# SahakyanLab/GenomeAssembler_dev

Measured on AMD Instinct MI355X. Metric: k-mers built+scored/sec, higher is better.
Workload: dtype u64 keys / u32 counts / f64 scores; 1 GPU; cfg2 (configs[2]): 100 x 50000 bp segments per GPU, 150 bp reads at 50x, k=31, build + breakage scoring of all contigs; mode=segments, segments_total=100, distinct_kmers_rank0=3843627, parallelism=segments sharded over 1 GPU(s), no collective

## Files before the change

genomeassembler_dev_amd/csrc/kernels.h:

```cpp
#pragma once
#include <hip/hip_runtime.h>
#include <stdint.h>

#include "device_utils.h"
#include "keyops.h"

struct ReadSet {
    const u64* words;
    const u64* read_off;
    const u64* seg_read_off;
    const u32* seg_tile_start;
    const uint4* tile_info;
    u32 fixed_len;
    u32 n_segments;
};

__device__ __forceinline__ void read_span(const ReadSet& rs, u64 r, u64* p0, u32* len) {
    if (rs.fixed_len) { *p0 = rs.read_off ? rs.read_off[r] : r * rs.fixed_len; *len = rs.fixed_len; }
    else { const u64 a = rs.read_off[r]; *p0 = a; *len = (u32)(rs.read_off[r + 1] - a); }
}

struct GraphView {
    const void* dk_key;
    const u32* dstart;
// ... 7 lines not shown
__device__ __forceinline__ u32 graph_lower_bound(const GraphView& gv, u32 seg, const K& t, u32* bucket_hi) {
    const K* dk = reinterpret_cast<const K*>(gv.dk_key);
    const u32 nb = 1u << gv.bbits;
    const int low = 2 * gv.k - gv.bbits;
    const u32 gb = seg * nb + (gv.bbits ? kfield(t, low) : 0u);
    uint2 dd;
    __builtin_memcpy(&dd, gv.dstart + gb, 8);
    const u32 base = dd.x;
    *bucket_hi = dd.y;
    const int bshift = low > gv.fbits ? low - gv.fbits : 0;
    const u32 nbin = 1u << gv.fbits;
    const u16* f = gv.fdir + (u64)gb * (nbin + 1) + (kfield(t, bshift) & (nbin - 1));
    u32 ff;
    __builtin_memcpy(&ff, f, 4);
    u32 lo = base + (ff & 0xFFFFu);
    u32 hi = base + (ff >> 16);
    if (hi > *bucket_hi) hi = *bucket_hi;
    if (lo > hi) lo = hi;
    while (hi - lo > 4) {
        const u32 m = (lo + hi) >> 1;
        if (kless(dk[m], t)) lo = m + 1;
        else hi = m;
    }
    while (lo < hi && kless(dk[lo], t)) ++lo;
    return lo;
}

struct PathSet {
    const u64* words;
    const u64* p_off;
    const u32* seg_path_off;
    u32 n_segments;
};

#define GASM_KT 16
#define GASM_SCORE_PATH_CAP 6144
#define GASM_TBL 4096
#define GASM_TBL_LIMIT 2816

__global__ void k_pack_ascii(const u8* ascii, u64 nbases_host, const u64* nbases_dev, u64* words, u32* err);
#define GASM_TILE_WG 512
template <class K> __global__ void k_tile_hist(ReadSet rs, const uint4* tinfo, int k, int bbits, u32 g, u32 n_tiles, ushort4* tcnt);
__global__ void k_tile_scan(ReadSet rs, int bbits, u32 padm, const ushort4* tcnt, u32* toff, u32* hist, u32* flags);
template <class TO> __global__ void k_scan_excl(const u32* in, TO* out, u32 n);
__global__ void k_copy_u64(const u64* a, u64* b, u32 n);
template <class K>
__global__ void k_bucket_scatter(ReadSet rs, const uint4* tinfo, int k, int bbits, u32 g, u32 padm, u32 n_tiles, const u64* bstart, const u32* toff,
                                 const ushort4* tcnt, K* keys, u64 scratch);
#define GASM_RT_MAX 16
template <class K>
__global__ void k_bucket_partition(ReadSet rs, const uint4* tinfo, int k, int bbits, u32 g, u32 padm, u32 n_tiles, const u64* bstart, u32* cursor,
                                   K* keys, u64 scratch, u32* flags);
template <class K, int TBL>
__global__ void k_bucket_dedup(K* keys, u32* mult, const u64* bstart, const u32* blen, u32* bucket_d, u32* overflow, u16* fdir, int low_bits, int dbg,
                               unsigned long long* stamps, u32* dstart);
#define GASM_BUCKET_MAX 65535
template <class K>
__global__ void k_bucket_dedup_multi(const K* keys, K* keys_out, u32* mult, const u64* bstart, u32* bucket_d, u32* overflow, u16* fdir, int low_bits);
template <class K>
__global__ void k_bucket_gather(const K* keys, const u32* mult, const u64* bstart, const u32* dstart, K* dk_key, u32* dk_cnt, u32* claim, u8* eflag,
                                u32* flags);
template <class K> __global__ void k_edge_target(GraphView gv, u32 n_segments, u32 chunks, u32* tgt, u32* claim);
__global__ void k_edge_multi(GraphView gv, u32 n_segments, u32 chunks, const u32* tgt, const u32* claim, u8* eflag);
template <class K>
__global__ void k_node_flags(GraphView gv, u32 n_segments, u32 chunks, const u32* claim, u8* eflag, u64* link, u32* clen);
__global__ void k_edge_next(GraphView gv, u32 n_segments, u32 chunks, const u32* tgt, const u8* eflag, u32* nxt, u64* link);
__global__ void k_link_jump(GraphView gv, u32 n_segments, u32 chunks, u64* link, const u32* prev_active, u32* active, int jumps, const u32* nxt,
                            u32* clen);
__global__ void k_rank_rulers(GraphView gv, u32 n_segments, u32 chunks, u64* link, u32* rtab, u32 rshift, u32* flags);
__global__ void k_rank_lds(GraphView gv, const u32* rtab, u64* link, int max_rounds, u32 rshift, u32 lds_entries, u32* flags);
__global__ void k_chain_len(const u32* nxt, const u64* link, u32* clen, const u32* n_edges_p);
__global__ void k_contig_scan(GraphView gv, const u8* eflag, const u32* clen, u32* e_cid, u64* e_coff, u32* seg_ncontig,
                              u64* seg_cbases, u32* done, u32* seg_cstart, u64* seg_bstart, const u32* flags, u32* report, u32 ticket);
__global__ void k_contig_place(GraphView gv, const u8* eflag, const u32* seg_cstart, const u64* seg_bstart, u32* e_cid, u64* e_coff,
                               u64* c_off, u32 n_segments, u32 chunks);
template <class K>
__global__ void k_contig_emit(GraphView gv, const u64* link, const u32* nxt, const u64* e_coff, u8* out, u32 n_segments, u32 chunks);

template <class K>
__global__ void k_pack_runs(const K* keys, const u32* mult, const u64* bstart, const u32* bucket_d, const u32* gb_list, const u64* dst_off, K* out_keys,
                            u32* out_cnt);
template <class K, int TBL>
__global__ void k_bucket_merge(const K* in_keys, const u32* in_cnt, const u64* run_off, const u32* run_len, u32 n_src, K* out_keys, u32* out_cnt,
                               const u64* bstart, u32* bucket_d, u32* overflow, u16* fdir, int low_bits, const u64* src_base);
__global__ void k_repack_reads(const u64* src, const u64* dir, u64* words_out);
__global__ void k_piece_positions(const u64* piece_first, const u64* piece_word_off, u32 n_pieces, u64 n_reads, u32 fixed_len, u64* pos);
__global__ void k_slice_last(const u32* a, const u64* off, u32 n, u32* out);

__global__ void k_chain_expand(const u64* cwords, const u64* c_off, const u64* sig_off, const u32* elem_contig, const u32* elem_skip, const u64* elem_pos,
                               const u64* out_off, u32 n_scaffolds, u64* out, u64 n_words);
struct ChainSigs {
    const u64* sig_off;
    const u32* elem_contig;
    const u32* elem_skip;
    const u64* elem_pos;
};
__global__ void k_str_bitonic(const u64* words, const u64* off, u32* idx, u32 n_pow2, u32 kk, u32 j, ChainSigs cs);
__global__ void k_str_bitonic_block(const u64* words, const u64* off, u32* idx, u32 n_pow2, u32 kk, u32 j0, ChainSigs cs);
__global__ void k_str_adjacent_eq(const u64* words, const u64* off, const u32* idx, u32 n, u8* same_as_prev, ChainSigs cs);
__global__ void k_unpack_ascii(const u64* words, u64 nbases, u8* out);
__global__ void k_guided_chain(PathSet ps, const unsigned long long* fx, int k, u32* g_next, u32* g_prev, u32* dbg_order);
__global__ void k_asm_match(const u64* cwords, const u64* c_off, u32 n, int k, u8* match, u8* row_any, u8* level_any);
__global__ void k_asm_merge(const u32* perm, u32 rows, u32 n, int k, const u32* clen, const u8* match, const u8* row_any, const u8* level_any,
                            const u64* cwords, const u64* c_off, u32* out_next, u8* out_ov, u32* out_heads, u32* out_nchains, u8* need_host);

__global__ void k_sim_weights(const u64* gwords, const u64* gbase, const u64* woff, u32 n_segments, int kmer, const long long* fixw, u64* w);
template <class T> __global__ void k_seg_scan_incl(T* a, const u64* off);
__global__ void k_sim_draw(const u64* cum, const u64* woff, const u64* doff, const u64* glen, u64 seed, u32 read_len, u32* start, u32* keep);
// ... 47 lines not shown
```

genomeassembler_dev_amd/csrc/kernels_build.hip:

```cpp
#include "device_utils.h"
#include "keyops.h"
#include "kernels.h"
#include "dedup_order.h"

typedef unsigned long long u64x2 __attribute__((ext_vector_type(2)));

typedef unsigned int u32x4nt __attribute__((ext_vector_type(4)));
#ifndef GASM_NO_NT
__device__ __forceinline__ uint4 stream_load16(const uint4* p) {
    const u32x4nt v = __builtin_nontemporal_load(reinterpret_cast<const u32x4nt*>(p));
    return make_uint4(v.x, v.y, v.z, v.w);
}
#define GASM_STREAM_LOAD(p) stream_load16(p)
#define GASM_STREAM_STORE(v, p) __builtin_nontemporal_store((v), (p))
#else
#define GASM_STREAM_LOAD(p) (*(p))
#define GASM_STREAM_STORE(v, p) (*(p) = (v))
#endif

__global__ void __launch_bounds__(GASM_WG) k_pack_ascii(const u8* __restrict__ ascii, u64 nbases_host, const u64* __restrict__ nbases_dev,
                                                        u64* __restrict__ words, u32* __restrict__ err) {
    const u64 nbases = nbases_dev ? *nbases_dev : nbases_host;
    const u64 nwords = (nbases + 31) / 32 + 4;
    bool ok = true;
// ... 437 lines not shown

#define GASM_SLOT_LOCKED 0xFFFFFFFFu

__device__ __forceinline__ u64x2 lds_load128(const void* p) {
    __asm__ volatile("" ::: "memory");
    return *reinterpret_cast<const u64x2*>(p);
}
__device__ __forceinline__ uint4 lds_load128u(const void* p) {
    __asm__ volatile("" ::: "memory");
    return *reinterpret_cast<const uint4*>(p);
}

template <int TBL>
__device__ __forceinline__ bool dedup_step(u64* t_key, u32* t_cnt, u32* n_distinct, u64 key, u32& set) {
    constexpr u32 NSETS = TBL / 2;
    const u64x2 c = lds_load128(&t_key[2 * set]);
    int slot = c.x == key ? 0 : c.y == key ? 1 : -1;
    if (slot < 0) {
        const int emp = c.x == GASM_EMPTY64 ? 0 : c.y == GASM_EMPTY64 ? 1 : -1;
        if (emp < 0) { set = (set + 1) & (NSETS - 1); return false; }
        const u64 old = atomicCAS(reinterpret_cast<unsigned long long*>(&t_key[2 * set + emp]), (unsigned long long)GASM_EMPTY64,
                                  (unsigned long long)key);
        if (old == GASM_EMPTY64) atomicAdd(n_distinct, 1u);
        else if (old != key) return false;
        slot = emp;
    }
    atomicAdd(&t_cnt[2 * set + slot], 1u);
    return true;
}
template <int TBL>
__device__ __forceinline__ bool dedup_step(K128* t_key, u32* t_cnt, u32* n_distinct, const K128& key, u32& set) {
    constexpr u32 NSETS = TBL / 2;
    __asm__ volatile("" ::: "memory");
    const uint2 c = *reinterpret_cast<const uint2*>(&t_cnt[2 * set]);
    const u32 cc[2] = {c.x, c.y};
#pragma unroll
    for (int q = 0; q < 2; ++q) {
        if (cc[q] == GASM_SLOT_LOCKED) return false;
        if (cc[q] == 0) {
            if (atomicCAS(&t_cnt[2 * set + q], 0u, GASM_SLOT_LOCKED) != 0u) return false;
            t_key[2 * set + q] = key;
            __builtin_amdgcn_fence(__ATOMIC_RELEASE, "workgroup");
            __hip_atomic_store(&t_cnt[2 * set + q], 1u, __ATOMIC_RELAXED, __HIP_MEMORY_SCOPE_WORKGROUP);
            atomicAdd(n_distinct, 1u);
            return true;
        }
        const u64x2 kq = lds_load128(&t_key[2 * set + q]);
        if (kq.x == key.hi && kq.y == key.lo) { atomicAdd(&t_cnt[2 * set + q], 1u); return true; }
    }
    set = set + 1 >= NSETS - 1 ? 0u : set + 1;
    return false;
}

#ifndef GASM_DEDUP_NLD
#define GASM_DEDUP_NLD 3
#endif
#ifndef GASM_DEDUP_NLDW
#define GASM_DEDUP_NLDW 6
#endif
#ifndef GASM_DEDUP_WGS
#define GASM_DEDUP_WGS 6
#endif
__device__ __forceinline__ void publish_u32(u32* p, u32 v) { __hip_atomic_store(p, v, __ATOMIC_RELAXED, __HIP_MEMORY_SCOPE_AGENT); }
__device__ __forceinline__ void publish_u64(u64* p, u64 v) { __hip_atomic_store(p, v, __ATOMIC_RELAXED, __HIP_MEMORY_SCOPE_AGENT); }
__device__ __forceinline__ bool count_in_last(u32* done) {
    __asm__ volatile("s_waitcnt vmcnt(0)" ::: "memory");
    return __hip_atomic_fetch_add(done, 1u, __ATOMIC_RELAXED, __HIP_MEMORY_SCOPE_AGENT) == gridDim.x - 1;
}

__device__ __forceinline__ void dedup_last_scan(const u32* __restrict__ bucket_d, u32* __restrict__ dstart, u32 n, u32* __restrict__ done, u32* s_word,
                                                u32* s_waves ) {
    if (!dstart) return;
    __syncthreads();
    if (threadIdx.x == 0) *s_word = count_in_last(done) ? 1u : 0u;
    __syncthreads();
    if (!*s_word) return;
    const u32 per = (n + GASM_WG - 1) / GASM_WG, a = min(n, threadIdx.x * per), b = min(n, a + per);
    u32 sum = 0;
    for (u32 i = a; i < b; ++i) sum += __hip_atomic_load(&bucket_d[i], __ATOMIC_RELAXED, __HIP_MEMORY_SCOPE_AGENT);
    const u32 inc = wave_incl_scan(sum);
    __syncthreads();
    if ((threadIdx.x & 63) == 63) s_waves[threadIdx.x >> 6] = inc;
    __syncthreads();
    u32 ex = inc - sum, tot = 0;
    for (u32 w = 0; w < GASM_WG / 64; ++w) { const u32 t = s_waves[w]; if (w < (threadIdx.x >> 6)) ex += t; tot += t; }
    for (u32 i = a; i < b; ++i) { dstart[i] = ex; ex += __hip_atomic_load(&bucket_d[i], __ATOMIC_RELAXED, __HIP_MEMORY_SCOPE_AGENT); }
    if (threadIdx.x == 0) dstart[n] = tot;
}

template <class K, int TBL>
__global__ void __launch_bounds__(GASM_WG, TBL == 4096 ? 3 : sizeof(K) == 8 ? GASM_DEDUP_WGS : 4)
k_bucket_dedup(K* __restrict__ keys, u32* __restrict__ mult, const u64* __restrict__ bstart, const u32* __restrict__ blen, u32* __restrict__ bucket_d,
               u32* __restrict__ overflow, u16* __restrict__ fdir, int low_bits, int dbg, unsigned long long* __restrict__ stamps,
               u32* __restrict__ dstart) {
    constexpr int LIMIT = TBL / 16 * 11;
    constexpr int BINS = TBL / 4;
    constexpr int LOG_TBL = TBL == 4096 ? 12 : 11;
    constexpr bool WIDE = sizeof(K) == 16;
    constexpr int LOG_SETS = LOG_TBL - 1;
    constexpr u32 NSETS = 1u << LOG_SETS;
    static_assert(TBL == 4096 || TBL == 2048, "table size");
    __shared__ __align__(32) K t_key[TBL];
    __shared__ __align__(16) u32 t_cnt[TBL];
    u32 *s_tmp, *w_distinct, *w_overflow;
    if constexpr (WIDE) {
        s_tmp = reinterpret_cast<u32*>(&t_key[TBL - 2]);
        w_distinct = &t_cnt[TBL - 2];
        w_overflow = &t_cnt[TBL - 1];
    } else {
        __shared__ u32 s_tmp_narrow[8];
        s_tmp = s_tmp_narrow;
        w_distinct = &s_tmp_narrow[4];
        w_overflow = &s_tmp_narrow[5];
    }
    static_assert((TBL - LIMIT) * sizeof(K) >= 2 * BINS * sizeof(u32), "the bins must fit behind the sorted entries");
    u32* const s_start = reinterpret_cast<u32*>(t_key + LIMIT);
    u32* const s_cur = s_start + BINS;
    unsigned long long tph = stamps ? wall_clock64() : 0ull;
    auto phase = [&](int i) {
        if (stamps && threadIdx.x == 0) { const unsigned long long t = wall_clock64(); atomicAdd(&stamps[i], t - tph); tph = t; }
    };
    const u32 bucket = blockIdx.x;
    const u64 beg = bstart[bucket], end = bstart[bucket + 1];
    u64 n = end - beg;
    if (blen) {
        const u64 len = blen[bucket];
        if (len > n) {
            for (u32 i = threadIdx.x; i <= (u32)BINS; i += GASM_WG) fdir[(u64)bucket * (BINS + 1) + i] = 0;
            if (threadIdx.x == 0) publish_u32(&bucket_d[bucket], 0u);
            dedup_last_scan(bucket_d, dstart, gridDim.x, overflow + 8, s_tmp + 7, s_tmp);
            return;
        }
        n = len;
    }
    const u32 warm = (u32)(dbg >> 2) & 3u;
    for (u32 i = threadIdx.x; i < TBL; i += GASM_WG) { t_key[i] = key_empty<K>(); t_cnt[i] = 0; }
    if (!WIDE && threadIdx.x == 0) { *w_distinct = 0; *w_overflow = 0; s_tmp[6] = 0; }
    __syncthreads();
    phase(0);
    constexpr int NLD = WIDE ? GASM_DEDUP_NLDW : TBL == 2048 ? GASM_DEDUP_NLD : 4;
    constexpr int KPL = NLD * 16 / sizeof(K);
    const u64 nch = n * sizeof(K) / 16;
    const uint4* src = reinterpret_cast<const uint4*>(keys + beg);
    if (dbg & 16) src = reinterpret_cast<const uint4*>(keys + bstart[bucket & 7u]);
    uint4 v[NLD];
    auto fetch = [&](u64 c) {
#pragma unroll
        for (int q = 0; q < NLD; ++q) v[q] = c + (u64)q * GASM_WG < nch ? GASM_STREAM_LOAD(&src[c + (u64)q * GASM_WG]) : make_uint4(~0u, ~0u, ~0u, ~0u);
    };
    if (threadIdx.x < nch) fetch(threadIdx.x);
    for (u64 c = threadIdx.x; c < nch; c += NLD * GASM_WG) {
        if (c == (u64)threadIdx.x + NLD * GASM_WG) phase(1);
        K kx[KPL];
        if constexpr (WIDE) {
#pragma unroll
            for (int q = 0; q < NLD; ++q) { kx[q].hi = (u64)v[q].x | ((u64)v[q].y << 32); kx[q].lo = (u64)v[q].z | ((u64)v[q].w << 32); }
        } else {
#pragma unroll
            for (int q = 0; q < NLD; ++q) { kx[2 * q] = (u64)v[q].x | ((u64)v[q].y << 32); kx[2 * q + 1] = (u64)v[q].z | ((u64)v[q].w << 32); }
        }
        if (c + NLD * GASM_WG < nch) fetch(c + NLD * GASM_WG);
        if ((dbg & 3) == 1) { u64 x = 0; for (int q = 0; q < KPL; ++q) x ^= khash(kx[q]); if (x == 0x1234567) *w_overflow = 1; continue; }
        if (__hip_atomic_load(w_distinct, __ATOMIC_RELAXED, __HIP_MEMORY_SCOPE_WORKGROUP) > (u32)LIMIT) { *w_overflow = 1; break; }
        if constexpr (!WIDE) {
            if (c < (u64)warm * NLD * GASM_WG) {
#pragma unroll
                for (int q = 0; q < KPL; ++q) {
                    const u64 key = kx[q];
                    if (kis_filler(key)) continue;
                    u32 st = khash(key) >> (32 - LOG_SETS);
                    bool ok = false;
                    for (u32 probe = 0; probe < 8 * NSETS && !ok; ++probe) ok = dedup_step<TBL>(t_key, t_cnt, w_distinct, key, st);
                    if (!ok) *w_overflow = 1;
                }
                continue;
            }
            u32 missed = 0;
            {
                u32 set[KPL];
                u64x2 c[KPL];
#pragma unroll
                for (int q = 0; q < KPL; ++q) {
                    set[q] = khash(kx[q]) >> (32 - LOG_SETS);
                    c[q] = lds_load128(&t_key[2 * set[q]]);
                }
#pragma unroll
                for (int q = 0; q < KPL; ++q) {
                    const u64 key = kx[q];
                    if (kis_filler(key)) continue;
                    const int slot = c[q].x == key ? 0 : c[q].y == key ? 1 : -1;
                    if (slot >= 0) atomicAdd(&t_cnt[2 * set[q] + slot], 1u);
                    else missed |= 1u << q;
                }
            }
            while (missed) {
                const u32 q = (u32)__builtin_ctz(missed);
                missed &= missed - 1;
                u64 key = kx[0];
#pragma unroll
                for (u32 e = 1; e < (u32)KPL; ++e) if (e == q) key = kx[e];
                u32 st = khash(key) >> (32 - LOG_SETS);
                bool ok = false;
                for (u32 probe = 0; probe < 8 * NSETS && !ok; ++probe) ok = dedup_step<TBL>(t_key, t_cnt, w_distinct, key, st);
                if (!ok) *w_overflow = 1;
            }
        } else {
            u32 set[KPL];
            uint2 cn[KPL];
            u64x2 k0[KPL], k1[KPL];
#pragma unroll
            for (int q = 0; q < KPL; ++q) {
                set[q] = min(khash(kx[q]) >> (32 - LOG_SETS), NSETS - 2);
                __asm__ volatile("" ::: "memory");
                cn[q] = *reinterpret_cast<const uint2*>(&t_cnt[2 * set[q]]);
                k0[q] = lds_load128(&t_key[2 * set[q]]);
                k1[q] = lds_load128(&t_key[2 * set[q] + 1]);
            }
            u32 missed = 0;
#pragma unroll
            for (int q = 0; q < KPL; ++q) {
                const K128 key = kx[q];
                if (kis_filler(key)) continue;
                const bool r0 = cn[q].x != 0 && cn[q].x != GASM_SLOT_LOCKED, r1 = cn[q].y != 0 && cn[q].y != GASM_SLOT_LOCKED;
                if (r0 && k0[q].x == key.hi && k0[q].y == key.lo) atomicAdd(&t_cnt[2 * set[q]], 1u);
                else if (r0 && r1 && k1[q].x == key.hi && k1[q].y == key.lo) atomicAdd(&t_cnt[2 * set[q] + 1], 1u);
                else missed |= 1u << q;
            }
            while (missed) {
                const u32 q = (u32)__builtin_ctz(missed);
                missed &= missed - 1;
                K128 key = kx[0];
#pragma unroll
                for (u32 e = 1; e < (u32)KPL; ++e) if (e == q) key = kx[e];
                u32 st = min(khash(key) >> (32 - LOG_SETS), NSETS - 2);
                bool ok = false;
                for (u32 probe = 0; probe < 8 * NSETS && !ok; ++probe) ok = dedup_step<TBL>(t_key, t_cnt, w_distinct, key, st);
                if (!ok) *w_overflow = 1;
            }
        }
    }
    phase(2);
    __syncthreads();
    phase(3);
    if (*w_overflow || *w_distinct > (u32)LIMIT) {
        for (u32 i = threadIdx.x; i <= (u32)BINS; i += GASM_WG) fdir[(u64)bucket * (BINS + 1) + i] = 0;
        if (threadIdx.x == 0) { atomicOr(overflow, 1u); publish_u32(&bucket_d[bucket], 0u); }
        dedup_last_scan(bucket_d, dstart, gridDim.x, overflow + 8, s_tmp + 7, s_tmp);
        return;
    }
    const u32 d = *w_distinct;
    if ((dbg & 3) == 1 || (dbg & 3) == 2) { if (threadIdx.x == 0) publish_u32(&bucket_d[bucket], d); dedup_last_scan(bucket_d, dstart, gridDim.x, overflow + 8, s_tmp + 7, s_tmp); return; }
    dedup_order<K, TBL, true>(t_key, t_cnt, s_start, s_cur, s_tmp, fdir, bucket, low_bits, d);
    phase(4);
    for (u32 i = threadIdx.x; i < d; i += GASM_WG) { keys[beg + i] = t_key[i]; mult[beg + i] = t_cnt[i]; }
    if (threadIdx.x == 0) publish_u32(&bucket_d[bucket], d);
    phase(5);
    if (stamps && threadIdx.x == 0) stamps[8 + 3 * (u64)blockIdx.x + 1] = wall_clock64();
    dedup_last_scan(bucket_d, dstart, gridDim.x, overflow + 8, s_tmp + 7, s_tmp);
}
template __global__ void k_bucket_dedup<u64, 4096>(u64*, u32*, const u64*, const u32*, u32*, u32*, u16*, int, int, unsigned long long*, u32*);
template __global__ void k_bucket_dedup<u64, 2048>(u64*, u32*, const u64*, const u32*, u32*, u32*, u16*, int, int, unsigned long long*, u32*);
template __global__ void k_bucket_dedup<K128, 2048>(K128*, u32*, const u64*, const u32*, u32*, u32*, u16*, int, int, unsigned long long*, u32*);

template <class K>
__global__ void __launch_bounds__(GASM_WG) k_bucket_dedup_multi(const K* __restrict__ keys, K* __restrict__ keys_out, u32* __restrict__ mult,
                                                                const u64* __restrict__ bstart, u32* __restrict__ bucket_d,
                                                                u32* __restrict__ overflow, u16* __restrict__ fdir, int low_bits) {
    constexpr int TBL = 4096, LIMIT = TBL / 16 * 11, BINS = TBL / 4, LOG_SETS = 11, LOG_BINS = 10;
    constexpr u32 NSETS = 1u << LOG_SETS;
    __shared__ __align__(32) K t_key[TBL];
    __shared__ __align__(16) u32 t_cnt[TBL];
    __shared__ u32 s_start[BINS];
    __shared__ u32 s_cur[BINS];
    __shared__ u32 s_tmp[8];
    const u32 bucket = blockIdx.x;
    const u64 beg = bstart[bucket], n = bstart[bucket + 1] - beg;
    const int bin_bits = low_bits < LOG_BINS ? low_bits : LOG_BINS;
    const int r_max = low_bits < 16 ? low_bits : 16;
    u16* const fd = fdir + (u64)bucket * (BINS + 1);
    auto give_up = [&]() {
        for (u32 i = threadIdx.x; i <= (u32)BINS; i += GASM_WG) fd[i] = 0;
        if (threadIdx.x == 0) { atomicOr(overflow, 1u); bucket_d[bucket] = 0; }
    };
    for (int r = 0;; ++r) {
        if (r > r_max) { give_up(); return; }
        const u32 npass = 1u << r;
        u32 total = 0;
        bool fits = true;
        for (u32 p = 0; p < npass; ++p) {
            for (u32 i = threadIdx.x; i < TBL; i += GASM_WG) { t_key[i] = key_empty<K>(); t_cnt[i] = 0; }
            for (u32 i = threadIdx.x; i < BINS; i += GASM_WG) s_start[i] = 0;
            if (threadIdx.x == 0) { s_tmp[4] = 0; s_tmp[5] = 0; s_tmp[6] = 0; }
            __syncthreads();
            for (u64 i = threadIdx.x; i < n; i += GASM_WG) {
                const K key = keys[beg + i];
                if (kis_filler(key)) continue;
                if (r && (kfield(key, low_bits - r) & (npass - 1)) != p) continue;
                if (__hip_atomic_load(&s_tmp[4], __ATOMIC_RELAXED, __HIP_MEMORY_SCOPE_WORKGROUP) > (u32)LIMIT) break;
                u32 st = khash(key) >> (32 - LOG_SETS);
                bool ok = false;
                for (u32 probe = 0; probe < 8 * NSETS && !ok; ++probe) ok = dedup_step<TBL>(t_key, t_cnt, &s_tmp[4], key, st);
                if (!ok) s_tmp[5] = 1;
            }
            __syncthreads();
            const u32 d = s_tmp[4];
            if (s_tmp[5] || d > (u32)LIMIT) { fits = false; break; }
            if (total + d > GASM_BUCKET_MAX) { give_up(); return; }
            u32 lo, hi;
            if (r <= bin_bits) { lo = p << (bin_bits - r); hi = (p + 1) << (bin_bits - r); }
            else { lo = p >> (r - bin_bits); hi = (p & ((1u << (r - bin_bits)) - 1u)) ? lo : lo + 1; }
            dedup_order<K, TBL, false, true>(t_key, t_cnt, s_start, s_cur, s_tmp, fdir, bucket, low_bits, d, total, lo, hi);
            for (u32 i = threadIdx.x; i < d; i += GASM_WG) { keys_out[beg + total + i] = t_key[i]; mult[beg + total + i] = t_cnt[i]; }
            total += d;
            __syncthreads();
        }
// ... 413 lines not shown
```

genomeassembler_dev_amd/csrc/keyops.h:

```cpp
#pragma once
#include "device_utils.h"

struct __attribute__((aligned(16))) K128 {
    u64 hi, lo;
};

template <class K> __device__ __forceinline__ K key_empty();
template <> __device__ __forceinline__ u64 key_empty<u64>() { return GASM_EMPTY64; }
template <> __device__ __forceinline__ K128 key_empty<K128>() { return K128{GASM_EMPTY64, GASM_EMPTY64}; }
template <class K> __device__ __forceinline__ K key_from_u64(u64 v);
template <> __device__ __forceinline__ u64 key_from_u64<u64>(u64 v) { return v; }
template <> __device__ __forceinline__ K128 key_from_u64<K128>(u64 v) { return K128{0, v}; }

template <class K> __device__ __forceinline__ K key_filler(u32 bkt, int bshift);
__device__ __forceinline__ bool kis_filler(u64 a) { return (a >> 63) != 0; }

__device__ __forceinline__ bool keq(u64 a, u64 b) { return a == b; }
__device__ __forceinline__ bool keq(const K128& a, const K128& b) { return a.hi == b.hi && a.lo == b.lo; }
__device__ __forceinline__ bool kless(u64 a, u64 b) { return a < b; }
__device__ __forceinline__ bool kless(const K128& a, const K128& b) { return a.hi < b.hi || (a.hi == b.hi && a.lo < b.lo); }
__device__ __forceinline__ bool kis_empty(u64 a) { return a == GASM_EMPTY64; }
__device__ __forceinline__ bool kis_empty(const K128& a) { return (a.hi & a.lo) == GASM_EMPTY64; }

__device__ __forceinline__ bool kis_filler(const K128& a) { return (a.hi >> 63) != 0; }

__device__ __forceinline__ u64 kshr(u64 a, int s) { return a >> s; }
__device__ __forceinline__ K128 kshr(const K128& a, int s) {
    if (s == 0) return a;
    if (s >= 64) return K128{0, a.hi >> (s - 64)};
    return K128{a.hi >> s, (a.lo >> s) | (a.hi << (64 - s))};
}
__device__ __forceinline__ u64 kshl(u64 a, int s) { return a << s; }
__device__ __forceinline__ K128 kshl(const K128& a, int s) {
    if (s == 0) return a;
    if (s >= 64) return K128{a.lo << (s - 64), 0};
    return K128{(a.hi << s) | (a.lo >> (64 - s)), a.lo << s};
}
__device__ __forceinline__ u64 kor(u64 a, u64 b) { return a | b; }
__device__ __forceinline__ K128 kor(const K128& a, const K128& b) { return K128{a.hi | b.hi, a.lo | b.lo}; }
__device__ __forceinline__ u64 klowbits(u64 a, int bits) { return bits >= 64 ? a : (a & ((1ull << bits) - 1)); }
__device__ __forceinline__ K128 klowbits(const K128& a, int bits) {
    if (bits >= 128) return a;
    if (bits >= 64) return K128{bits == 64 ? 0 : (a.hi & ((1ull << (bits - 64)) - 1)), a.lo};
    return K128{0, a.lo & ((1ull << bits) - 1)};
}
template <> __device__ __forceinline__ u64 key_filler<u64>(u32 bkt, int bshift) { return (1ull << 63) | ((u64)bkt << bshift); }
template <> __device__ __forceinline__ K128 key_filler<K128>(u32 bkt, int bshift) {
    const K128 b = kshl(K128{0, (u64)bkt}, bshift);
    return K128{b.hi | (1ull << 63), b.lo};
}
__device__ __forceinline__ u32 kfield(u64 a, int s) { return (u32)(a >> s); }
__device__ __forceinline__ u32 kfield(const K128& a, int s) { return (u32)kshr(a, s).lo; }
__device__ __forceinline__ u32 klow2(u64 a) { return (u32)a & 3u; }
__device__ __forceinline__ u32 klow2(const K128& a) { return (u32)a.lo & 3u; }

__device__ __forceinline__ u32 khash(u64 a) {
    const u32 lo = (u32)a, hi = (u32)(a >> 32);
    u32 x = lo ^ __builtin_amdgcn_alignbit(hi, hi, 19);
    x ^= x >> 17;
    return __umul24(x, 0xB5297Au) ^ __umul24(x >> 8, 0x68E31Du);
}
__device__ __forceinline__ u32 khash(const K128& a) { return hash64(a.lo ^ (a.hi * 0xD6E8FEB86659FD93ull)); }

template <class K> __device__ __forceinline__ K kmer_key_at(const u64* __restrict__ w, u64 p, int k);
template <> __device__ __forceinline__ u64 kmer_key_at<u64>(const u64* __restrict__ w, u64 p, int k) { return window32(w, p) >> (64 - 2 * k); }
template <> __device__ __forceinline__ K128 kmer_key_at<K128>(const u64* __restrict__ w, u64 p, int k) {
    const K128 win{window32(w, p), window32(w, p + 32)};
    return kshr(win, 128 - 2 * k);
}

__device__ __forceinline__ u64 funnel64(u64 x, u64 y, u32 o) { return (x << o) | ((y >> 1) >> (63 - o)); }
template <u32 J> __device__ __forceinline__ u32 word_at(u32 hi, u32 lo) {
    if constexpr (J == 0) return hi;
    else return __builtin_amdgcn_alignbit(hi, lo, 32 - 2 * J);
}

template <class K> struct Roll;
template <> struct Roll<u64> {
    u64 w0, w1, w2;
    u32 s;
    __device__ __forceinline__ void load(const u64* __restrict__ w, u64 p) {
        const u64 i = p >> 5;
        w0 = w[i]; w1 = w[i + 1]; w2 = w[i + 2];
        s = (u32)(p & 31) << 1;
    }
    struct Win {
        u32 d3, d2, d1;
        template <u32 J> __device__ __forceinline__ u64 top() const { return ((u64)word_at<J>(d3, d2) << 32) | word_at<J>(d2, d1); }
        template <u32 J> __device__ __forceinline__ u32 top_hi() const { return word_at<J>(d3, d2); }
        template <u32 J> __device__ __forceinline__ u64 key(int k) const { return top<J>() >> (64 - 2 * k); }
    };
    __device__ __forceinline__ Win prep() const {
        const u64 hi = funnel64(w0, w1, s), lo = funnel64(w1, w2, s);
        return Win{(u32)(hi >> 32), (u32)hi, (u32)(lo >> 32)};
    }
    __device__ __forceinline__ void touch() const { __asm__ volatile("" :: "v"(w0), "v"(w1), "v"(w2)); }
    template <int N> __device__ __forceinline__ void wait_all_but() {
        __asm__ volatile("s_waitcnt vmcnt(%3)" : "+v"(w0), "+v"(w1), "+v"(w2) : "n"(N) : "memory");
    }
};
template <> struct Roll<K128> {
    u64 w0, w1, w2, w3;
    u32 s;
    __device__ __forceinline__ void load(const u64* __restrict__ w, u64 p) {
        const u64 i = p >> 5;
        w0 = w[i]; w1 = w[i + 1]; w2 = w[i + 2]; w3 = w[i + 3];
        s = (u32)(p & 31) << 1;
    }
    struct Win {
        u32 d5, d4, d3, d2, d1;
        template <u32 J> __device__ __forceinline__ u32 top_hi() const { return word_at<J>(d5, d4); }
        template <u32 J> __device__ __forceinline__ K128 key(int k) const {
            const K128 win{((u64)word_at<J>(d5, d4) << 32) | word_at<J>(d4, d3), ((u64)word_at<J>(d3, d2) << 32) | word_at<J>(d2, d1)};
            return kshr(win, 128 - 2 * k);
        }
// ... 15 lines not shown
```

genomeassembler_dev_amd/csrc/pipeline.hip:

```cpp
#include <atomic>
#include <chrono>
#include <thread>
#include "pipeline.h"

#include <algorithm>
#include <cmath>

__global__ void k_set_u64(u64* p, u64 v) { *p = v; }

__global__ void k_add_empty_reads(PathSet ps, const u64* __restrict__ seg_empty, u32* __restrict__ poscnt, u32* __restrict__ total) {
    const u32 seg = blockIdx.y;
    const u32 p = ps.seg_path_off[seg] + blockIdx.x * GASM_WG + threadIdx.x;
    if (p >= ps.seg_path_off[seg + 1]) return;
    const u32 e = (u32)seg_empty[seg];
    if (!e) return;
    if (ps.p_off[p + 1] > ps.p_off[p]) poscnt[ps.p_off[p]] += e;
    else total[p] += e;
}

struct Knobs {
    int dedup_tbl = 0, dbg_dedup = 0, padm = -1, scatter_wgs = 8, hist_wgs = 64, rank_rounds = 18, bbits_add = 0, ruler_shift = 0;
    bool rank_global = false, sync_build = false;
    int dedup_warm = 0;
    const char* stamps = nullptr;
// ... 473 lines not shown
        n_alloc = N + (u64)padm * rd.n_tiles * nb;
        GCHK(bs.d_keys.ensure((n_alloc + SCRATCH_KEYS) * KB));
        GCHK(bs.d_mult.ensure(n_alloc * 4));
        GCHK(bs.d_tcnt.ensure((size_t)rd.n_tiles * nb * 8 + 64));
        if (W == 1) {
            GLAUNCH(ctx, "k_tile_hist", k_tile_hist<u64>, dim3(grid_tiles), dim3(GASM_TILE_WG), (size_t)nb * 16, rs, rs.tile_info, k, bbits, g, rd.n_tiles,
                    bs.d_tcnt.as<ushort4>());
        } else {
            GLAUNCH(ctx, "k_tile_hist", k_tile_hist<K128>, dim3(grid_tiles), dim3(GASM_TILE_WG), (size_t)nb * 16, rs, rs.tile_info, k, bbits, g, rd.n_tiles,
                    bs.d_tcnt.as<ushort4>());
        }
        GLAUNCH(ctx, "k_tile_scan", k_tile_scan, dim3(S, std::max(1u, nb / 32u)), dim3(1024), 0, rs, bbits, padm, bs.d_tcnt.as<ushort4>(),
                bs.d_toff.as<u32>(), bs.d_hist.as<u32>(), bs.d_flags.as<u32>());
        GLAUNCH(ctx, "k_scan_excl", k_scan_excl<u64>, dim3(1), dim3(1024), 0, bs.d_hist.as<u32>(), bs.d_bstart.as<u64>(), nbt);
        const size_t lds = (size_t)(W == 1 ? 18 : 9) * GASM_TILE_WG * KB + (GASM_TILE_WG / 8) * KB + (size_t)nb * 24 + 96;
        const u32 grid_scatter = std::min<u32>(rd.n_tiles, (u32)ctx->n_cu * (u32)knobs().scatter_wgs);
        if (W == 1) {
            GLAUNCH(ctx, "k_bucket_scatter", k_bucket_scatter<u64>, dim3(grid_scatter), dim3(GASM_TILE_WG), lds, rs, rs.tile_info, k, bbits, g, padm, rd.n_tiles,
                    bs.d_bstart.as<u64>(), bs.d_toff.as<u32>(), bs.d_tcnt.as<ushort4>(), bs.d_keys.as<u64>(), n_alloc);
        } else {
            GLAUNCH(ctx, "k_bucket_scatter", k_bucket_scatter<K128>, dim3(grid_scatter), dim3(GASM_TILE_WG), lds, rs, rs.tile_info, k, bbits, g, padm, rd.n_tiles,
                    bs.d_bstart.as<u64>(), bs.d_toff.as<u32>(), bs.d_tcnt.as<ushort4>(), bs.d_keys.as<K128>(), n_alloc);
        }
    }
    if (bs.ev_before_dedup) HIPCHK(hipStreamWaitEvent(ctx->stream, bs.ev_before_dedup, 0));
    unsigned long long* d_stamps = nullptr;
    static DBuf stamp_buf;
    if (knobs().stamps) {
        int o1 = 0, o2 = 0, o3 = 0, o4 = 0;
        const size_t lds_stage = (size_t)(W == 1 ? 18 : 9) * GASM_TILE_WG * KB + (GASM_TILE_WG / 8) * KB;
        (void)hipOccupancyMaxActiveBlocksPerMultiprocessor(&o1, k_bucket_dedup<u64, 2048>, GASM_WG, 0);
        (void)hipOccupancyMaxActiveBlocksPerMultiprocessor(&o2, k_bucket_dedup<u64, 4096>, GASM_WG, 0);
        (void)hipOccupancyMaxActiveBlocksPerMultiprocessor(&o3, k_bucket_scatter<u64>, GASM_TILE_WG, lds_stage + (size_t)nb * 24 + 96);
        (void)hipOccupancyMaxActiveBlocksPerMultiprocessor(&o4, k_bucket_partition<u64>, GASM_TILE_WG, lds_stage + (size_t)nb * 40 + 96);
        fprintf(stderr, "[occupancy API] dedup<2048> %d  dedup<4096> %d  scatter %d  partition %d blocks/CU\n", o1, o2, o3, o4);
        GCHK(stamp_buf.ensure(64 + (size_t)nbt * 24));
        HIPCHK(hipMemsetAsync(stamp_buf.p, 0, 64 + (size_t)nbt * 24, ctx->stream));
        d_stamps = stamp_buf.as<unsigned long long>();
    }
    const int dbg_d = knobs().dbg_dedup | (knobs().dedup_warm << 2);
    const bool scan_in_dedup = !bs.multi_pass && nbt <= 16384 && env_int("GASM_SCAN_IN_DEDUP", 1) != 0;
    u32* const d_scan_out = scan_in_dedup ? bs.d_dstart.as<u32>() : nullptr;
    bs.fbits = (bs.small_tbl && !bs.multi_pass) ? 9 : 10;
    GCHK(bs.d_fdir.ensure((size_t)nbt * ((1u << bs.fbits) + 1) * 2));
    if (bs.multi_pass) {
        GCHK(bs.d_keys2.ensure(n_alloc * KB));
        if (W == 2) GLAUNCH(ctx, "k_bucket_dedup_multi", k_bucket_dedup_multi<K128>, dim3(nbt), dim3(GASM_WG), 0, bs.d_keys.as<K128>(), bs.d_keys2.as<K128>(),
                            bs.d_mult.as<u32>(), bs.d_bstart.as<u64>(), bs.d_bucket_d.as<u32>(), bs.d_flags.as<u32>(), bs.d_fdir.as<u16>(), 2 * k - bbits);
        else GLAUNCH(ctx, "k_bucket_dedup_multi", k_bucket_dedup_multi<u64>, dim3(nbt), dim3(GASM_WG), 0, bs.d_keys.as<u64>(), bs.d_keys2.as<u64>(),
                     bs.d_mult.as<u32>(), bs.d_bstart.as<u64>(), bs.d_bucket_d.as<u32>(), bs.d_flags.as<u32>(), bs.d_fdir.as<u16>(), 2 * k - bbits);
        HIPCHK(hipMemcpyAsync(bs.d_keys.p, bs.d_keys2.p, n_alloc * KB, hipMemcpyDeviceToDevice, ctx->stream));
    } else if (W == 2) {
        GLAUNCH(ctx, "k_bucket_dedup", (k_bucket_dedup<K128, 2048>), dim3(nbt), dim3(GASM_WG), 0, bs.d_keys.as<K128>(), bs.d_mult.as<u32>(),
                bs.d_bstart.as<u64>(), d_blen, bs.d_bucket_d.as<u32>(), bs.d_flags.as<u32>(), bs.d_fdir.as<u16>(), 2 * k - bbits, dbg_d, d_stamps, d_scan_out);
    } else if (bs.small_tbl) {
        GLAUNCH(ctx, "k_bucket_dedup", (k_bucket_dedup<u64, 2048>), dim3(nbt), dim3(GASM_WG), 0, bs.d_keys.as<u64>(), bs.d_mult.as<u32>(),
                bs.d_bstart.as<u64>(), d_blen, bs.d_bucket_d.as<u32>(), bs.d_flags.as<u32>(), bs.d_fdir.as<u16>(), 2 * k - bbits, dbg_d, d_stamps, d_scan_out);
    } else {
        GLAUNCH(ctx, "k_bucket_dedup", (k_bucket_dedup<u64, 4096>), dim3(nbt), dim3(GASM_WG), 0, bs.d_keys.as<u64>(), bs.d_mult.as<u32>(),
                bs.d_bstart.as<u64>(), d_blen, bs.d_bucket_d.as<u32>(), bs.d_flags.as<u32>(), bs.d_fdir.as<u16>(), 2 * k - bbits, dbg_d, d_stamps, d_scan_out);
    }
    if (d_stamps) {
        std::vector<unsigned long long> hv(8 + (size_t)nbt * 3);
        HIPCHK(hipMemcpyAsync(hv.data(), d_stamps, hv.size() * 8, hipMemcpyDeviceToHost, ctx->stream));
        HIPCHK(hipStreamSynchronize(ctx->stream));
        const unsigned long long* h = hv.data();
        if (FILE* f = fopen(knobs().stamps, "wb")) { fwrite(hv.data(), 8, hv.size(), f); fclose(f); }
        fprintf(stderr, "[dedup stamps, 100 MHz ticks per workgroup] init %.1f  first-iter %.1f  stream %.1f  barrier %.1f  order %.1f  writeback %.1f\n",
                (double)h[0] / nbt, (double)h[1] / nbt, (double)h[2] / nbt, (double)h[3] / nbt, (double)h[4] / nbt, (double)h[5] / nbt);
    }
    if (!scan_in_dedup) GLAUNCH(ctx, "k_scan_excl", k_scan_excl<u32>, dim3(1), dim3(1024), 0, bs.d_bucket_d.as<u32>(), bs.d_dstart.as<u32>(), nbt);
    return GASM_OK;
}

static int alloc_graph(BuildState& bs, u32 S) {
    const u64 D = std::max<u64>(bs.D_cap, 1);
    const size_t KB = 8 * (size_t)bs.words;
    if (D >= 0xFFFFFFF0ull) { gasm_set_error("more than 2^32 distinct k-mers possible in one batch: split it"); return GASM_ERR_CAPACITY; }
    GCHK(bs.d_dk_key.ensure(D * KB));
    GCHK(bs.d_dk_cnt.ensure(D * 4));
    GCHK(bs.d_eflag.ensure(D));
    GCHK(bs.d_nxt.ensure(D * 4));
    GCHK(bs.d_link.ensure(D * 8));
    GCHK(bs.d_clen.ensure(D * 4));
    GCHK(bs.d_ecid.ensure(D * 4));
    GCHK(bs.d_ecoff.ensure(D * 8));
    GCHK(bs.d_rtab.ensure((D / 2 + S + 2) * 4));
    GCHK(bs.d_seg_cbases.ensure((size_t)S * 8 + (size_t)S * 4));
    GCHK(bs.d_seg_cstart.ensure(((size_t)S + 1) * 4));
    GCHK(bs.d_seg_bstart.ensure(((size_t)S + 1) * 8));
    bs.bases_cap = D * (u64)bs.k;
    if (bs.bases_cap >= 0xFFFFFFF0ull) { gasm_set_error("contigs could exceed 2^32 bases: split the batch"); return GASM_ERR_CAPACITY; }
    GCHK(bs.d_c_off.ensure((D + 1) * 8));
    GCHK(bs.d_contig_ascii.ensure(bs.bases_cap + 64));
    return GASM_OK;
}

int launch_graph(gasm_ctx* ctx, u32 S, BuildState& bs) {
    const int W = bs.words, bbits = bs.bbits;
    const u32 nb = 1u << bbits, nbt = S * nb;
    GCHK(alloc_graph(bs, S));
    u32* const d_claim = bs.d_nxt.as<u32>();
    if (W == 1) {
        GLAUNCH(ctx, "k_bucket_gather", k_bucket_gather<u64>, dim3(nbt), dim3(GASM_WG), 0, bs.d_keys.as<u64>(), bs.d_mult.as<u32>(),
                bs.d_bstart.as<u64>(), bs.d_dstart.as<u32>(), bs.d_dk_key.as<u64>(), bs.d_dk_cnt.as<u32>(), d_claim, bs.d_eflag.as<u8>(), bs.d_flags.as<u32>());
    } else {
        GLAUNCH(ctx, "k_bucket_gather", k_bucket_gather<K128>, dim3(nbt), dim3(GASM_WG), 0, bs.d_keys.as<K128>(), bs.d_mult.as<u32>(),
                bs.d_bstart.as<u64>(), bs.d_dstart.as<u32>(), bs.d_dk_key.as<K128>(), bs.d_dk_cnt.as<u32>(), d_claim, bs.d_eflag.as<u8>(), bs.d_flags.as<u32>());
    }
    return launch_graph_dense(ctx, S, bs);
}

static int launch_graph_dense(gasm_ctx* ctx, u32 S, BuildState& bs) {
    GasmRange range("gasm:graph (degrees, list ranking, contigs)");
    const int W = bs.words;
    u32* const d_claim = bs.d_nxt.as<u32>();
    u32* const d_seg_ncontig = reinterpret_cast<u32*>(bs.d_seg_cbases.as<u64>() + S);
    u32* const d_fl = bs.d_flags.as<u32>();
    const GraphView gv = graph_view(bs);
    const u32 nb = 1u << bs.bbits;
    const u32 est = std::max<u32>(1, (u32)std::min<u64>(bs.maxD_est, bs.maxD_cap));
    const u32 dchunks = (u32)ceil_div_u64(est, GASM_WG);
// ... 717 lines not shown
```

Baseline: 223.0 billion k-mers/s.

## Pad dedup tails with bucket-local filler key and cheapen k-mer hash

Padding loads in the bucket dedup kernel now use a filler key that belongs to the current bucket instead of all-ones. This lets the per-key filler check be removed from the hot loop, and the filler's table entry is dropped once after streaming. The u64 and 128-bit hashes are replaced with a cheaper single multiply, and the hit-path count increment uses direct byte-offset addressing. The patch also adds debug counters for probe misses gated on stamps. Risks are weaker hash distribution causing more probe misses or overflow, and correctness depending on the filler removal and the adjusted LIMIT+1 threshold.

```diff
diff --git a/genomeassembler_dev_amd/csrc/kernels.h b/genomeassembler_dev_amd/csrc/kernels.h
--- a/genomeassembler_dev_amd/csrc/kernels.h
+++ b/genomeassembler_dev_amd/csrc/kernels.h
@@ -83,8 +83,8 @@
 __global__ void k_bucket_partition(ReadSet rs, const uint4* tinfo, int k, int bbits, u32 g, u32 padm, u32 n_tiles, const u64* bstart, u32* cursor,
                                    K* keys, u64 scratch, u32* flags);
 template <class K, int TBL>
-__global__ void k_bucket_dedup(K* keys, u32* mult, const u64* bstart, const u32* blen, u32* bucket_d, u32* overflow, u16* fdir, int low_bits, int dbg,
-                               unsigned long long* stamps, u32* dstart);
+__global__ void k_bucket_dedup(K* keys, u32* mult, const u64* bstart, const u32* blen, u32* bucket_d, u32* overflow, u16* fdir, int low_bits, u32 bmask,
+                               int dbg, unsigned long long* stamps, u32* dstart);
 #define GASM_BUCKET_MAX 65535
 template <class K>
 __global__ void k_bucket_dedup_multi(const K* keys, K* keys_out, u32* mult, const u64* bstart, u32* bucket_d, u32* overflow, u16* fdir, int low_bits);
diff --git a/genomeassembler_dev_amd/csrc/kernels_build.hip b/genomeassembler_dev_amd/csrc/kernels_build.hip
--- a/genomeassembler_dev_amd/csrc/kernels_build.hip
+++ b/genomeassembler_dev_amd/csrc/kernels_build.hip
@@ -513,6 +513,29 @@
     return false;
 }
 
+template <int TBL>
+__device__ __forceinline__ void dedup_drop_filler(u64* t_key, u32* t_cnt, u32* w_distinct, u64 fk) {
+    constexpr u32 NSETS = TBL / 2;
+    u32 set = khash(fk) >> (32 - (TBL == 4096 ? 11 : 10));
+    for (u32 p = 0; p < NSETS; ++p, set = (set + 1) & (NSETS - 1)) {
+        const u64x2 c = lds_load128(&t_key[2 * set]);
+        if (c.x == fk || c.y == fk) { t_key[2 * set + (c.x == fk ? 0 : 1)] = GASM_EMPTY64; --*w_distinct; return; }
+        if (c.x == GASM_EMPTY64 || c.y == GASM_EMPTY64) return;
+    }
+}
+template <int TBL>
+__device__ __forceinline__ void dedup_drop_filler(K128* t_key, u32* t_cnt, u32* w_distinct, const K128& fk) {
+    constexpr u32 NSETS = TBL / 2;
+    u32 set = min(khash(fk) >> (32 - (TBL == 4096 ? 11 : 10)), NSETS - 2);
+    for (u32 p = 0; p < NSETS; ++p, set = set + 1 >= NSETS - 1 ? 0u : set + 1) {
+#pragma unroll
+        for (u32 q = 0; q < 2; ++q) {
+            if (t_cnt[2 * set + q] == 0) return;
+            if (keq(t_key[2 * set + q], fk)) { t_cnt[2 * set + q] = 0; --*w_distinct; return; }
+        }
+    }
+}
+
 #ifndef GASM_DEDUP_NLD
 #define GASM_DEDUP_NLD 3
 #endif
@@ -552,7 +575,7 @@
 template <class K, int TBL>
 __global__ void __launch_bounds__(GASM_WG, TBL == 4096 ? 3 : sizeof(K) == 8 ? GASM_DEDUP_WGS : 4)
 k_bucket_dedup(K* __restrict__ keys, u32* __restrict__ mult, const u64* __restrict__ bstart, const u32* __restrict__ blen, u32* __restrict__ bucket_d,
-               u32* __restrict__ overflow, u16* __restrict__ fdir, int low_bits, int dbg, unsigned long long* __restrict__ stamps,
+               u32* __restrict__ overflow, u16* __restrict__ fdir, int low_bits, u32 bmask, int dbg, unsigned long long* __restrict__ stamps,
                u32* __restrict__ dstart) {
     constexpr int LIMIT = TBL / 16 * 11;
     constexpr int BINS = TBL / 4;
@@ -598,16 +621,24 @@
     for (u32 i = threadIdx.x; i < TBL; i += GASM_WG) { t_key[i] = key_empty<K>(); t_cnt[i] = 0; }
     if (!WIDE && threadIdx.x == 0) { *w_distinct = 0; *w_overflow = 0; s_tmp[6] = 0; }
     __syncthreads();
+    if (!WIDE && stamps) {
+        if (threadIdx.x == 0) { s_tmp[0] = 0; s_tmp[1] = 0; }
+        __syncthreads();
+    }
     phase(0);
+    const K fk = key_filler<K>(bucket & bmask, low_bits);
     constexpr int NLD = WIDE ? GASM_DEDUP_NLDW : TBL == 2048 ? GASM_DEDUP_NLD : 4;
     constexpr int KPL = NLD * 16 / sizeof(K);
     const u64 nch = n * sizeof(K) / 16;
     const uint4* src = reinterpret_cast<const uint4*>(keys + beg);
     if (dbg & 16) src = reinterpret_cast<const uint4*>(keys + bstart[bucket & 7u]);
     uint4 v[NLD];
+    uint4 pad;
+    if constexpr (WIDE) pad = make_uint4((u32)fk.hi, (u32)(fk.hi >> 32), (u32)fk.lo, (u32)(fk.lo >> 32));
+    else pad = make_uint4((u32)fk, (u32)(fk >> 32), (u32)fk, (u32)(fk >> 32));
     auto fetch = [&](u64 c) {
 #pragma unroll
-        for (int q = 0; q < NLD; ++q) v[q] = c + (u64)q * GASM_WG < nch ? GASM_STREAM_LOAD(&src[c + (u64)q * GASM_WG]) : make_uint4(~0u, ~0u, ~0u, ~0u);
+        for (int q = 0; q < NLD; ++q) v[q] = c + (u64)q * GASM_WG < nch ? GASM_STREAM_LOAD(&src[c + (u64)q * GASM_WG]) : pad;
     };
     if (threadIdx.x < nch) fetch(threadIdx.x);
     for (u64 c = threadIdx.x; c < nch; c += NLD * GASM_WG) {
@@ -622,13 +653,12 @@
         }
         if (c + NLD * GASM_WG < nch) fetch(c + NLD * GASM_WG);
         if ((dbg & 3) == 1) { u64 x = 0; for (int q = 0; q < KPL; ++q) x ^= khash(kx[q]); if (x == 0x1234567) *w_overflow = 1; continue; }
-        if (__hip_atomic_load(w_distinct, __ATOMIC_RELAXED, __HIP_MEMORY_SCOPE_WORKGROUP) > (u32)LIMIT) { *w_overflow = 1; break; }
+        if (__hip_atomic_load(w_distinct, __ATOMIC_RELAXED, __HIP_MEMORY_SCOPE_WORKGROUP) > (u32)LIMIT + 1) { *w_overflow = 1; break; }
         if constexpr (!WIDE) {
             if (c < (u64)warm * NLD * GASM_WG) {
 #pragma unroll
                 for (int q = 0; q < KPL; ++q) {
                     const u64 key = kx[q];
-                    if (kis_filler(key)) continue;
                     u32 st = khash(key) >> (32 - LOG_SETS);
                     bool ok = false;
                     for (u32 probe = 0; probe < 8 * NSETS && !ok; ++probe) ok = dedup_step<TBL>(t_key, t_cnt, w_distinct, key, st);
@@ -647,13 +677,12 @@
                 }
 #pragma unroll
                 for (int q = 0; q < KPL; ++q) {
-                    const u64 key = kx[q];
-                    if (kis_filler(key)) continue;
-                    const int slot = c[q].x == key ? 0 : c[q].y == key ? 1 : -1;
-                    if (slot >= 0) atomicAdd(&t_cnt[2 * set[q] + slot], 1u);
+                    const bool h0 = c[q].x == kx[q], h1 = c[q].y == kx[q];
+                    if (h0 || h1) atomicAdd(reinterpret_cast<u32*>(reinterpret_cast<unsigned char*>(t_cnt) + ((set[q] << 3) | (h0 ? 0u : 4u))), 1u);
                     else missed |= 1u << q;
                 }
             }
+            if (stamps) atomicAdd(&s_tmp[c == threadIdx.x ? 1 : 0], (u32)__builtin_popcount(missed));
             while (missed) {
                 const u32 q = (u32)__builtin_ctz(missed);
                 missed &= missed - 1;
@@ -681,12 +710,12 @@
 #pragma unroll
             for (int q = 0; q < KPL; ++q) {
                 const K128 key = kx[q];
-                if (kis_filler(key)) continue;
                 const bool r0 = cn[q].x != 0 && cn[q].x != GASM_SLOT_LOCKED, r1 = cn[q].y != 0 && cn[q].y != GASM_SLOT_LOCKED;
                 if (r0 && k0[q].x == key.hi && k0[q].y == key.lo) atomicAdd(&t_cnt[2 * set[q]], 1u);
                 else if (r0 && r1 && k1[q].x == key.hi && k1[q].y == key.lo) atomicAdd(&t_cnt[2 * set[q] + 1], 1u);
                 else missed |= 1u << q;
             }
+            if (stamps) atomicAdd(&stamps[c == threadIdx.x ? 7 : 6], (unsigned long long)__builtin_popcount(missed));
             while (missed) {
                 const u32 q = (u32)__builtin_ctz(missed);
                 missed &= missed - 1;
@@ -701,6 +730,9 @@
         }
     }
     phase(2);
+    __syncthreads();
+    if (!WIDE && stamps && threadIdx.x == 0) { atomicAdd(&stamps[6], (unsigned long long)s_tmp[0]); atomicAdd(&stamps[7], (unsigned long long)s_tmp[1]); }
+    if (threadIdx.x == 0 && !*w_overflow) dedup_drop_filler<TBL>(t_key, t_cnt, w_distinct, fk);
     __syncthreads();
     phase(3);
     if (*w_overflow || *w_distinct > (u32)LIMIT) {
@@ -719,9 +751,9 @@
     if (stamps && threadIdx.x == 0) stamps[8 + 3 * (u64)blockIdx.x + 1] = wall_clock64();
     dedup_last_scan(bucket_d, dstart, gridDim.x, overflow + 8, s_tmp + 7, s_tmp);
 }
-template __global__ void k_bucket_dedup<u64, 4096>(u64*, u32*, const u64*, const u32*, u32*, u32*, u16*, int, int, unsigned long long*, u32*);
-template __global__ void k_bucket_dedup<u64, 2048>(u64*, u32*, const u64*, const u32*, u32*, u32*, u16*, int, int, unsigned long long*, u32*);
-template __global__ void k_bucket_dedup<K128, 2048>(K128*, u32*, const u64*, const u32*, u32*, u32*, u16*, int, int, unsigned long long*, u32*);
+template __global__ void k_bucket_dedup<u64, 4096>(u64*, u32*, const u64*, const u32*, u32*, u32*, u16*, int, u32, int, unsigned long long*, u32*);
+template __global__ void k_bucket_dedup<u64, 2048>(u64*, u32*, const u64*, const u32*, u32*, u32*, u16*, int, u32, int, unsigned long long*, u32*);
+template __global__ void k_bucket_dedup<K128, 2048>(K128*, u32*, const u64*, const u32*, u32*, u32*, u16*, int, u32, int, unsigned long long*, u32*);
 
 template <class K>
 __global__ void __launch_bounds__(GASM_WG) k_bucket_dedup_multi(const K* __restrict__ keys, K* __restrict__ keys_out, u32* __restrict__ mult,
diff --git a/genomeassembler_dev_amd/csrc/keyops.h b/genomeassembler_dev_amd/csrc/keyops.h
--- a/genomeassembler_dev_amd/csrc/keyops.h
+++ b/genomeassembler_dev_amd/csrc/keyops.h
@@ -56,11 +56,10 @@
 
 __device__ __forceinline__ u32 khash(u64 a) {
     const u32 lo = (u32)a, hi = (u32)(a >> 32);
-    u32 x = lo ^ __builtin_amdgcn_alignbit(hi, hi, 19);
-    x ^= x >> 17;
-    return __umul24(x, 0xB5297Au) ^ __umul24(x >> 8, 0x68E31Du);
+    const u32 x = lo ^ __builtin_amdgcn_alignbit(hi, lo, 24) ^ (hi >> 14);
+    return __umul24(x, 0x9E3779u);
 }
-__device__ __forceinline__ u32 khash(const K128& a) { return hash64(a.lo ^ (a.hi * 0xD6E8FEB86659FD93ull)); }
+__device__ __forceinline__ u32 khash(const K128& a) { return khash(a.lo ^ ((a.hi << 29) | (a.hi >> 35))); }
 
 template <class K> __device__ __forceinline__ K kmer_key_at(const u64* __restrict__ w, u64 p, int k);
 template <> __device__ __forceinline__ u64 kmer_key_at<u64>(const u64* __restrict__ w, u64 p, int k) { return window32(w, p) >> (64 - 2 * k); }
diff --git a/genomeassembler_dev_amd/csrc/pipeline.hip b/genomeassembler_dev_amd/csrc/pipeline.hip
--- a/genomeassembler_dev_amd/csrc/pipeline.hip
+++ b/genomeassembler_dev_amd/csrc/pipeline.hip
@@ -549,13 +549,13 @@
         HIPCHK(hipMemcpyAsync(bs.d_keys.p, bs.d_keys2.p, n_alloc * KB, hipMemcpyDeviceToDevice, ctx->stream));
     } else if (W == 2) {
         GLAUNCH(ctx, "k_bucket_dedup", (k_bucket_dedup<K128, 2048>), dim3(nbt), dim3(GASM_WG), 0, bs.d_keys.as<K128>(), bs.d_mult.as<u32>(),
-                bs.d_bstart.as<u64>(), d_blen, bs.d_bucket_d.as<u32>(), bs.d_flags.as<u32>(), bs.d_fdir.as<u16>(), 2 * k - bbits, dbg_d, d_stamps, d_scan_out);
+                bs.d_bstart.as<u64>(), d_blen, bs.d_bucket_d.as<u32>(), bs.d_flags.as<u32>(), bs.d_fdir.as<u16>(), 2 * k - bbits, nb - 1, dbg_d, d_stamps, d_scan_out);
     } else if (bs.small_tbl) {
         GLAUNCH(ctx, "k_bucket_dedup", (k_bucket_dedup<u64, 2048>), dim3(nbt), dim3(GASM_WG), 0, bs.d_keys.as<u64>(), bs.d_mult.as<u32>(),
-                bs.d_bstart.as<u64>(), d_blen, bs.d_bucket_d.as<u32>(), bs.d_flags.as<u32>(), bs.d_fdir.as<u16>(), 2 * k - bbits, dbg_d, d_stamps, d_scan_out);
+                bs.d_bstart.as<u64>(), d_blen, bs.d_bucket_d.as<u32>(), bs.d_flags.as<u32>(), bs.d_fdir.as<u16>(), 2 * k - bbits, nb - 1, dbg_d, d_stamps, d_scan_out);
     } else {
         GLAUNCH(ctx, "k_bucket_dedup", (k_bucket_dedup<u64, 4096>), dim3(nbt), dim3(GASM_WG), 0, bs.d_keys.as<u64>(), bs.d_mult.as<u32>(),
-                bs.d_bstart.as<u64>(), d_blen, bs.d_bucket_d.as<u32>(), bs.d_flags.as<u32>(), bs.d_fdir.as<u16>(), 2 * k - bbits, dbg_d, d_stamps, d_scan_out);
+                bs.d_bstart.as<u64>(), d_blen, bs.d_bucket_d.as<u32>(), bs.d_flags.as<u32>(), bs.d_fdir.as<u16>(), 2 * k - bbits, nb - 1, dbg_d, d_stamps, d_scan_out);
     }
     if (d_stamps) {
         std::vector<unsigned long long> hv(8 + (size_t)nbt * 3);
@@ -565,6 +565,8 @@
         if (FILE* f = fopen(knobs().stamps, "wb")) { fwrite(hv.data(), 8, hv.size(), f); fclose(f); }
         fprintf(stderr, "[dedup stamps, 100 MHz ticks per workgroup] init %.1f  first-iter %.1f  stream %.1f  barrier %.1f  order %.1f  writeback %.1f\n",
                 (double)h[0] / nbt, (double)h[1] / nbt, (double)h[2] / nbt, (double)h[3] / nbt, (double)h[4] / nbt, (double)h[5] / nbt);
+        fprintf(stderr, "[dedup misses] keys that missed their home set: %llu in first iterations, %llu after (of %llu keys)\n", h[7], h[6],
+                (unsigned long long)N);
     }
     if (!scan_in_dedup) GLAUNCH(ctx, "k_scan_excl", k_scan_excl<u32>, dim3(1), dim3(1024), 0, bs.d_bucket_d.as<u32>(), bs.d_dstart.as<u32>(), nbt);
     return GASM_OK;
```

Result: no change. 224.3 billion k-mers/s, median of 6 (+0.6%).
